# ZikangXiong/mobrob

Measured on AMD Instinct MI355X. Metric: env-steps/sec (whole node), doggo PPO, higher is better.
Workload: dtype f32

## Files before the change

mobrob_amd/csrc/engine.hip:

```cpp
#include <hip/hip_runtime.h>
#include <rccl/rccl.h>
#include <dlfcn.h>

#include <algorithm>
#include <atomic>
#include <thread>
#include <cmath>
#include <cstdarg>
#include <cstdio>
#include <climits>
#include <cstring>
#include <ctime>
#include <cstdlib>
#include <string>
#include <vector>

#ifdef MOBROB_POISON_LDS
namespace mobrob {
__global__ __launch_bounds__(1024) void k_poison_lds() {
  extern __shared__ unsigned poison_words[];
  volatile unsigned* w = poison_words;
  for (int i = threadIdx.x; i < 160 * 256; i += 1024) w[i] = 0xFFFFFFFFu;
}
inline void poison_lds(hipStream_t st) {
// ... 155 lines not shown
  ncclComm_t comm = nullptr;
  int64_t allreduce_calls = 0, allreduce_bytes = 0;
  struct OneShot {
    char* xbuf = nullptr;
    size_t payload = 0;
    char* peer[kOneShotMaxRanks] = {nullptr};
    int world = 0, rank = -1;
    bool ready = false;
    unsigned long long seq = 0;
    int* error = nullptr;
    long long timeout_ticks = 0;
  } oneshot;
  double* norm_rec_sum = nullptr; int* norm_rec_t = nullptr; int* fold_idx_dev = nullptr;
  int fold_start[kMaxTensors + 1] = {0};
  bool use_norm_records = false;
  bool epoch_kernel_on = true;
  unsigned* epoch_bar = nullptr;
  float* epoch_consts = nullptr;
  int* epoch_idx = nullptr;
  char* epoch_stage = nullptr;
  int* epoch_err_host = nullptr;
  hipEvent_t epoch_ev = nullptr;
  int last_update_mode = 0;
  float* epoch_snap = nullptr;
  int rollout64_tile_max = 256;
  int pair64_min_tiles = 65;
  int split64_max_tiles = 64;
  float *Xg = nullptr, *actg = nullptr, *lpg = nullptr, *advg = nullptr, *retg = nullptr, *oldvg = nullptr;
  float *hp[kMaxHidden] = {nullptr}, *hv[kMaxHidden] = {nullptr}, *mu = nullptr, *vout = nullptr;
  float *dmu = nullptr, *dv = nullptr, *dzp[kMaxHidden] = {nullptr}, *dzv[kMaxHidden] = {nullptr};
// ... 205 lines not shown
                       int M, int Nn, int rows, GemmQueue* q = nullptr) {
  GemmOp o;
  GemmArgs& g = o.g;
  g.A = dY; g.B = X; g.C = dW; g.M = M; g.N = Nn; g.K = rows; g.lda = ldd; g.ldb = ldx; g.ldc = ldw;
  const int wtiles = cdiv(M, M <= 32 ? 32 : 64) * cdiv(Nn, (M <= 32 || Nn <= 32) ? 32 : 64);
  int ksplit = std::max(1, std::min(cdiv(rows, 64), cdiv(2048, wtiles)));
  g.kchunk = rup(cdiv(rows, ksplit), 8);
  o.ksplit = cdiv(rows, g.kchunk);
  o.mode = MODE_TN; o.epi = EPI_ATOMIC;
  if (q) q->push_back(o); else launch_op(e, o);
}

float* Pp(mobrob_ppo_engine* e, int t) { return e->params + e->offs[t]; }
float* Gp(mobrob_ppo_engine* e, int t) { return e->grads + e->offs[t]; }

void pack_x3_all(mobrob_ppo_engine* e) {
  if (e->fused.net[0].W2x == nullptr) return;
  PackX3Args a{};
  const int w1[2] = {T_PW1, T_VW1}, w2[2] = {T_PW2, T_VW2};
  int maxthreads = 0;
  for (int n = 0; n < 2; ++n) {
    const int i1 = 3 * n, i2 = 3 * n + 1, i3 = 3 * n + 2;
    a.W[i1] = Pp(e, w1[n]); a.N[i1] = FH; a.K[i1] = e->D; a.ld[i1] = e->D; a.NB[i1] = FH / 32; a.KS[i1] = e->Dp / 16; a.scale[i1] = kTanhScale;
    a.out[i1] = reinterpret_cast<unsigned short*>(const_cast<unsigned*>(e->fused.net[n].W1x));
    a.W[i2] = Pp(e, w2[n]); a.N[i2] = FH; a.K[i2] = FH; a.ld[i2] = FH; a.NB[i2] = FH / 32; a.KS[i2] = FH / 16; a.scale[i2] = kTanhScale;
    a.out[i2] = reinterpret_cast<unsigned short*>(const_cast<unsigned*>(e->fused.net[n].W2x));
    a.W[i3] = Pp(e, w2[n]); a.N[i3] = FH; a.K[i3] = FH; a.ld[i3] = FH; a.NB[i3] = FH / 32; a.KS[i3] = FH / 16; a.scale[i3] = 1.0f; a.trans[i3] = 1;
    a.out[i3] = reinterpret_cast<unsigned short*>(const_cast<unsigned*>(e->fused.net[n].W2bx));
    maxthreads = std::max(maxthreads, std::max(a.NB[i1] * a.KS[i1], a.NB[i2] * a.KS[i2]) * 512);
  }
  hipLaunchKernelGGL(k_pack_x3_multi, dim3(cdiv(maxthreads, 256), 6), dim3(256), 0, e->stream, a);
  if (e->fused.train_chain) {
    ChainPackArgs c{};
    const int w3[2] = {T_AW, T_VW};
    for (int n = 0; n < 2; ++n) {
      c.W1[n] = Pp(e, w1[n]); c.W2[n] = Pp(e, w2[n]); c.W3[n] = Pp(e, w3[n]);
      c.w1c[n] = reinterpret_cast<unsigned short*>(const_cast<unsigned*>(e->fused.net[n].W1c));
      c.w2c[n] = reinterpret_cast<unsigned short*>(const_cast<unsigned*>(e->fused.net[n].W2c));
      c.w2bc[n] = reinterpret_cast<unsigned short*>(const_cast<unsigned*>(e->fused.net[n].W2bc));
      c.w3c[n] = const_cast<float*>(e->fused.net[n].W3c); c.w3bc[n] = const_cast<float*>(e->fused.net[n].W3bc);
      c.head[n] = n == 0 ? e->A : 1;
    }
    c.D = e->D; c.Dp = e->Dp;
    hipLaunchKernelGGL(k_pack_chain, dim3(FH * FH / 256, 2), dim3(256), 0, e->stream, c);
  }
}

void repack(mobrob_ppo_engine* e) {
  auto pad = [&](const float* src, float* dst, int r, int c, int rp, int cp) {
    hipLaunchKernelGGL(k_pad_rows, dim3(cdiv(rp * cp, 256)), dim3(256), 0, e->stream, src, dst, r, c, rp, cp);
  };
  pad(Pp(e, T_PW1), e->pW1p, e->H1, e->D, e->H1, e->Dp);
  pad(Pp(e, T_VW1), e->vW1p, e->G1, e->D, e->G1, e->Dp);
  pad(Pp(e, T_AW), e->aWp, e->A, e->HL, e->Ap, e->HL);
  pad(Pp(e, T_VW), e->vWp, 1, e->GL, 8, e->GL);
  fused_repack(e->fused, e->params, e->offs, e->stream);
  pack_x3_all(e);
}

void forward_generic(mobrob_ppo_engine* e, const float* X, int rows, bool want_pi, float* mu_out, bool want_v,
                     float* v_out, bool keep_z = false) {
  GemmQueue qp, qv;
  if (want_pi) {
    linear_fwd(e, X, e->Dp, e->pW1p, e->Dp, Pp(e, e->tPB[0]), e->hp[0], e->Hp[0], rows, e->Hp[0], e->Dp, true, keep_z ? e->dzp[0] : nullptr, &qp);
    for (int l = 1; l < e->Lp; ++l)
      linear_fwd(e, e->hp[l - 1], e->Hp[l - 1], Pp(e, e->tPW[l]), e->Hp[l - 1], Pp(e, e->tPB[l]), e->hp[l], e->Hp[l], rows, e->Hp[l], e->Hp[l - 1], true,
                 keep_z ? e->dzp[l] : nullptr, &qp);
    linear_fwd(e, e->hp[e->Lp - 1], e->HL, e->aWp, e->HL, Pp(e, T_AB), mu_out, e->Ap, rows, e->A, e->HL, false, nullptr, &qp);
  }
  if (want_v) {
    linear_fwd(e, X, e->Dp, e->vW1p, e->Dp, Pp(e, e->tVB[0]), e->hv[0], e->Hv[0], rows, e->Hv[0], e->Dp, true, keep_z ? e->dzv[0] : nullptr, &qv);
    for (int l = 1; l < e->Lv; ++l)
      linear_fwd(e, e->hv[l - 1], e->Hv[l - 1], Pp(e, e->tVW[l]), e->Hv[l - 1], Pp(e, e->tVB[l]), e->hv[l], e->Hv[l], rows, e->Hv[l], e->Hv[l - 1], true,
                 keep_z ? e->dzv[l] : nullptr, &qv);
    linear_fwd(e, e->hv[e->Lv - 1], e->GL, e->vWp, e->GL, Pp(e, T_VB), v_out, 1, rows, 1, e->GL, false, nullptr, &qv);
  }
  run_queues(e, qp, qv, 1);
}

void forward(mobrob_ppo_engine* e, const float* X, int rows, bool want_pi, float* mu_out, bool want_v, float* v_out) {
  if (e->fused.enabled && fused_forward(e->fused, X, rows, want_pi, mu_out, e->Ap, want_v, v_out, e->stream)) return;
  forward_generic(e, X, rows, want_pi, mu_out, want_v, v_out);
}

int value_net_width_sum(const mobrob_ppo_engine* e) {
  int s = 0;
  for (int l = 0; l < e->Lv; ++l) s += e->Hv[l];
  return s;
}
ValueNetArgs value_net_args(mobrob_ppo_engine* e) {
  ValueNetArgs vn{};
  for (int l = 0; l < e->Lv; ++l) { vn.W[l] = Pp(e, e->tVW[l]); vn.b[l] = Pp(e, e->tVB[l]); vn.G[l] = e->Hv[l]; }
  vn.Wv = Pp(e, T_VW); vn.bv = Pp(e, T_VB);
  vn.L = e->Lv; vn.act = e->cfg.activation; vn.width_sum = value_net_width_sum(e);
  return vn;
// ... 19 lines not shown
void sde_resample(mobrob_ppo_engine* e, int r0, int n, uint32_t draw, const uint32_t* draw_base, bool single) {
  const int HLA = e->HL * e->A, per = cdiv(HLA, 4);
  hipLaunchKernelGGL(k_sde_resample, dim3(cdiv((n + (single ? 1 : 0)) * per, 256)), dim3(256), 0, e->stream, Pp(e, T_LOGSTD), HLA, e->A, e->sde_mode, r0, n,
                     eps_seed(e) ^ 0x5DE5DE5DE5DE5DEull, draw, draw_base, e->sde_E, single ? e->sde_E1 : (float*)nullptr);
}

void sde_variance(mobrob_ppo_engine* e, int rows, bool fresh_table, float* lat2 = nullptr) {
  if (fresh_table)
    hipLaunchKernelGGL(k_sde_std2, dim3(cdiv(e->HL * e->A, 256)), dim3(256), 0, e->stream, Pp(e, T_LOGSTD), e->HL, e->A, e->sde_mode, e->sde_S2);
  hipLaunchKernelGGL(k_sde_var, dim3(cdiv(rows, 4)), dim3(256), 0, e->stream, e->hp[e->Lp - 1], e->HL, e->sde_S2, rows, e->HL, e->A, e->sde_var, e->Ap,
                     lat2);
}

void act_rows(mobrob_ppo_engine* e, int t, int r0, int n, const float* eps_dev_or_null, uint32_t draw,
              const uint32_t* draw_base, float* clip_out = nullptr) {
  ProfScope ps(e, MOBROB_K_ACT);
  if (!clip_out) clip_out = e->clip_act + (size_t)r0 * e->A;
  const size_t row = (size_t)t * e->N + r0;
  const float* X = e->obs + row * e->Dp;
  if (e->fused.enabled) {
    FusedActArgs a{};
    a.X = X; a.rows = n; a.row0 = r0; a.want_pi = 1; a.want_v = 1; a.mu = nullptr; a.ldmu = e->Ap;
    a.v = e->values + row; a.sample = 1; a.A = e->A; a.log_std = Pp(e, T_LOGSTD); a.eps = eps_dev_or_null;
    a.seed = eps_seed(e); a.draw = draw; a.draw_base = draw_base; a.lo = (float)e->cfg.action_low; a.hi = (float)e->cfg.action_high;
    a.act_raw = e->actions + row * e->A; a.act_clip = clip_out; a.logp = e->logp + row;
    fused_launch_act(e->fused, a, e->stream);
    return;
  }
  forward(e, X, n, true, e->mu, true, e->values + row);
  if (e->sde) {
// ... 45 lines not shown
  return a;
}
template <class Args>
Args reduce_args(const mobrob_ppo_engine* e) {
  Args s{};
  s.slabs = e->fused.slabs; s.grads = e->grads; s.P = e->P;
  for (int i = 0; i < 14; ++i) s.offs[i] = e->offs[i];
  s.D = e->D; s.A = e->A; s.ent_coef = (float)e->cfg.ent_coef; s.sums = e->grads + e->P;
  s.rec_sum = e->use_norm_records ? e->norm_rec_sum : nullptr; s.rec_t = e->norm_rec_t;
  return s;
}
Slab64ReduceArgs slab64_reduce_args(const mobrob_ppo_engine* e) { return reduce_args<Slab64ReduceArgs>(e); }
SlabReduceArgs slab_reduce_args(const mobrob_ppo_engine* e) {
  SlabReduceArgs s = reduce_args<SlabReduceArgs>(e);
  s.slab_floats = e->fused.slab_floats; s.Dp = e->Dp; s.h16 = e->A <= 16;
  return s;
}
StatsArgs stats_args(const mobrob_ppo_engine* e) {
  StatsArgs st{};
  st.loss_sums = e->grads + e->P; st.log_std = e->params + e->offs[T_LOGSTD]; st.n_act = e->A; st.sde = e->sde;
  st.ent_coef = (float)e->cfg.ent_coef; st.vf_coef = (float)e->cfg.vf_coef;
  return st;
}
int fused_carve_packs(mobrob_ppo_engine* e) {
  FusedState& f = e->fused;
  const int H = f.H;
  const size_t nW1 = (size_t)(H / 32) * (e->Dp / 8) * 256, nW2 = (size_t)(H / 32) * (H / 8) * 256;
  const size_t nW3f = (size_t)(H / 8) * 256, nW3b = (size_t)(H / 32) * 4 * 256;
  const size_t nW3h = (size_t)(H / 16) * 256;
  const size_t per_net = nW1 + 2 * nW2 + nW3f + nW3h + nW3b + 2 * H;
// ... 59 lines not shown
        f.lds_chain_bytes = chain_lds_bytes(e->Dp);
      }
    }
    CHK(dalloc(e, &f.train_rec, (size_t)e->N * e->T * train_rec_width(e->A)));
    f.lds_bytes = fused_lds_bytes(e->Dp);
    f.lds_act_bytes = fused_lds_act_bytes(e->Dp);
  }
  return dalloc(e, &f.stamps, 32);
}
int build_norm_record_tables(mobrob_ppo_engine* e) {
  const FusedState& f = e->fused;
  const int nb = cdiv(f.slab_floats, 256);
  CHK(dalloc(e, &e->norm_rec_sum, (size_t)2 * nb * kNormRec));
  CHK(dalloc(e, &e->norm_rec_t, (size_t)2 * nb * kNormRec));
  CHK(dalloc(e, &e->fold_idx_dev, (size_t)2 * nb * kNormRec));
  const SlabReduceArgs s256 = slab_reduce_args(e);
  const Slab64ReduceArgs s64 = slab64_reduce_args(e);
  std::vector<std::vector<int>> per_tensor(13);
  for (int net = 0; net < 2; ++net)
    for (int b = 0; b < nb; ++b) {
      std::vector<int> recs;
      for (int w = 0; w < 4; ++w) {
        std::vector<int> wave;
        for (int l = 0; l < 64; ++l) {
          const int p = b * 256 + w * 64 + l;
          const int dst = p < f.slab_floats ? (f.H == 64 ? slab64_to_canonical(s64, net, p) : slab_to_canonical(s256, net, p)) : -1;
          const int t = tensor_of_canonical(e->offs, e->P, dst);
          if (t >= 0 && std::find(wave.begin(), wave.end(), t) == wave.end()) wave.push_back(t);
        }
        for (int t : wave)
// ... 826 lines not shown
}
int rollout_side_stream_init(mobrob_ppo_engine* e) {
  if (!e->vstream) {
    HIPC(hipStreamCreateWithFlags(&e->vstream, hipStreamNonBlocking));
    HIPC(hipEventCreateWithFlags(&e->ev_vdone, hipEventDisableTiming));
  }
  while ((int)e->ev_chunks.size() < e->T / 16 + 2) {
    hipEvent_t ev;
    HIPC(hipEventCreateWithFlags(&ev, hipEventDisableTiming));
    e->ev_chunks.push_back(ev);
  }
  return MOBROB_OK;
}

RolloutArgs rollout_args(mobrob_ppo_engine* e) {
  RolloutArgs a{};
  a.pi = e->fused.net[0];
  a.log_std = Pp(e, T_LOGSTD); a.seed = eps_seed(e);
  a.lo = (float)e->cfg.action_low; a.hi = (float)e->cfg.action_high;
  a.bt = BootArgs{Pp(e, T_VW1), Pp(e, T_VB1), Pp(e, T_VW2), Pp(e, T_VB2), Pp(e, T_VW), Pp(e, T_VB), e->G1, e->G2,
                  (float)e->cfg.gamma, e->term_val};
  a.N = e->N; a.D = e->D; a.A = e->A;
  a.obs = e->obs; a.actions = e->actions; a.logp = e->logp; a.rewards = e->rewards; a.es = e->es;
  a.term_obs = e->term_obs; a.trunc = e->trunc_dev; a.clip_act = e->clip_act;
  a.ep_len = e->ep_len; a.prev_dones = e->prev_dones; a.gstate = e->gstate[0]; a.ep_stats = e->ep_stats;
  return a;
}

bool wide_nets(const mobrob_ppo_engine* e) { return e->fused.H == FH; }
bool rollout64_tile_kernel(const mobrob_ppo_engine* e) { return cdiv(e->N, 32) <= e->rollout64_tile_max; }
// ... 144 lines not shown
    if (sp.kind == 1) {
      hipLaunchKernelGGL(k_env_reset, dim3(cdiv(N * per, 256)), dim3(256), 0, e->stream, env_seed_of(e), N, e->D, Dp, last,
                         e->ep_len);
    } else {
      hipLaunchKernelGGL(k_goal_env_reset, dim3(cdiv(N * per, 256)), dim3(256), 0, e->stream, env_seed_of(e), N, e->D, Dp,
                         sp.goal, e->gstate[0], last);
      HIPC(hipMemsetAsync(e->ep_stats, 0, kEpStatsDoubles * sizeof(double), e->stream));
      e->ep_ring_read = 0;
    }
    std::vector<float> ones(N, 1.0f);
    HIPC(hipMemcpyAsync(e->prev_dones, ones.data(), (size_t)N * 4, hipMemcpyHostToDevice, e->stream));
    HIPC(hipStreamSynchronize(e->stream));
    e->env_started = sp.kind;
  }
  e->rollout_ready = false; e->train_rec_valid = false;
  if (rollout_persistent_ok(e)) CHK(rollout_side_stream_init(e));
  bool use_graph = e->cfg.rollout_graph && e->T % 2 == 0 && !rollout_persistent_ok(e);
  if (use_graph && (e->ro_exec == nullptr || memcmp(&e->ro_spec, &sp, sizeof sp) != 0)) {
    HIPC(hipStreamSynchronize(e->stream));
    if (e->ro_exec) { (void)hipGraphExecDestroy(e->ro_exec); e->ro_exec = nullptr; }
    if (e->ro_graph) { (void)hipGraphDestroy(e->ro_graph); e->ro_graph = nullptr; }
    const bool prof = e->prof_on;
    e->prof_on = false;
    hipError_t be = hipStreamBeginCapture(e->stream, hipStreamCaptureModeThreadLocal);
    if (be != hipSuccess) {
      (void)hipGetLastError();
      e->prof_on = prof;
      e->cfg.rollout_graph = 0;
      use_graph = false;
    } else {
// ... 466 lines not shown
  if (!e->fused.enabled) generic_minibatch_grad(e, mb, start, B, inv_bg);
  else if (e->fused.H == 64) fused64_minibatch_grad(e, mb, start, B, inv_bg);
  else fused_minibatch_grad(e, mb, start, B, inv_bg);
  HIPC(hipGetLastError());
  e->grad_pending = true;
  return MOBROB_OK;
}

namespace {
void fill_adam_pack_args(mobrob_ppo_engine* e, AdamPackArgs& a) {
  a.p = e->params; a.g = e->grads; a.m = e->m; a.v = e->v; a.P = e->P;
  a.chunks = e->chunks_dev; a.partial = e->chunk_partial; a.nchunks = e->nchunks;
  if (e->use_norm_records) {
    a.partial = e->norm_rec_sum; a.fold_idx = e->fold_idx_dev;
    for (int i = 0; i <= kMaxTensors; ++i) a.fold_start[i] = e->fold_start[i];
  }
  a.max_norm = (float)e->cfg.max_grad_norm; a.beta1 = (float)e->cfg.adam_beta1; a.beta2 = (float)e->cfg.adam_beta2;
  a.eps = (float)e->cfg.adam_eps;
  for (int i = 0; i <= kMaxTensors; ++i) a.offs[i] = e->offs[i];
  a.ntens = e->ntens; a.two_by_two = e->Lp == 2 && e->Lv == 2; a.id_pw1 = T_PW1; a.id_vw1 = T_VW1; a.id_aw = T_AW; a.id_vw = T_VW; a.HL = e->HL; a.GL = e->GL;
  a.D = e->D; a.Dp = e->Dp; a.A = e->A; a.Ap = e->Ap; a.H1 = e->H1; a.H2 = e->H2; a.G1 = e->G1; a.G2 = e->G2;
  a.pW1p = e->pW1p; a.vW1p = e->vW1p; a.aWp = e->aWp; a.vWp = e->vWp;
  for (int n = 0; n < 2; ++n) {
    const bool on = e->fused.enabled;
    a.fW1f[n] = on ? (float*)e->fused.net[n].W1f : nullptr;
    a.fW2f[n] = on ? (float*)e->fused.net[n].W2f : nullptr;
    a.fW3f[n] = on ? (float*)e->fused.net[n].W3f : nullptr;
    const bool ch = on && e->fused.train_chain;
    a.fW2b[n] = on && !ch ? (float*)e->fused.net[n].W2b : nullptr;
    a.fW3b[n] = on && !ch ? (float*)e->fused.net[n].W3b : nullptr;
    a.fW3h[n] = (on && (n == 1 || e->fused.A <= 16)) ? (float*)e->fused.net[n].W3h : nullptr;
    a.fb1s[n] = on ? (float*)e->fused.net[n].b1s : nullptr;
    a.fb2s[n] = on ? (float*)e->fused.net[n].b2s : nullptr;
    const bool x3 = on && e->fused.train_x3;
    a.xW1[n] = x3 ? reinterpret_cast<unsigned short*>(const_cast<unsigned*>(e->fused.net[n].W1x)) : nullptr;
    a.xW2[n] = x3 ? reinterpret_cast<unsigned short*>(const_cast<unsigned*>(e->fused.net[n].W2x)) : nullptr;
    a.xW2b[n] = x3 && !ch ? reinterpret_cast<unsigned short*>(const_cast<unsigned*>(e->fused.net[n].W2bx)) : nullptr;
    a.cW1[n] = ch ? reinterpret_cast<unsigned short*>(const_cast<unsigned*>(e->fused.net[n].W1c)) : nullptr;
    a.cW2[n] = ch ? reinterpret_cast<unsigned short*>(const_cast<unsigned*>(e->fused.net[n].W2c)) : nullptr;
    a.cW2b[n] = ch ? reinterpret_cast<unsigned short*>(const_cast<unsigned*>(e->fused.net[n].W2bc)) : nullptr;
    a.cW3[n] = ch ? const_cast<float*>(e->fused.net[n].W3c) : nullptr;
    a.cW3b[n] = ch ? const_cast<float*>(e->fused.net[n].W3bc) : nullptr;
  }
}
}

namespace {
struct AdamStep { float step_size, bc2_sqrt; };
AdamStep next_adam_step(mobrob_ppo_engine* e) {
  e->adam_step++;
  const double bc1 = 1.0 - std::pow(e->cfg.adam_beta1, (double)e->adam_step), bc2 = 1.0 - std::pow(e->cfg.adam_beta2, (double)e->adam_step);
// ... 9 lines not shown
  st.inv_bg = 1.0f / (float)((int64_t)e->cur_count * e->cfg.world_size);
  if (!e->use_norm_records)
    hipLaunchKernelGGL(k_sqnorm_chunks, dim3(e->nchunks), dim3(256), 0, e->stream, e->grads, e->chunks_dev,
                       e->chunk_partial, st);
  return st;
}
int apply_adam(mobrob_ppo_engine* e, const StatsArgs& st) {
  const AdamStep step = next_adam_step(e);
  AdamPackArgs a{};
  fill_adam_pack_args(e, a);
  a.step_size = step.step_size; a.bc2_sqrt = step.bc2_sqrt;
  if (e->use_norm_records) a.st = st;
  a.stats_row = st.stats_row;
  a.loss_sums_zero = e->fused.enabled ? e->grads + e->P : nullptr;
  hipLaunchKernelGGL(k_adam_pack, dim3(cdiv(e->P, 256)), dim3(256), 0, e->stream, a);
  HIPC(hipGetLastError());
  e->grad_pending = false;
  return MOBROB_OK;
}
}

namespace {
int apply_checked(mobrob_ppo_engine* e, int32_t* stopped) {
  *stopped = 0;
  ProfScope ps(e, MOBROB_K_APPLY);
  const StatsArgs st = apply_norms(e);
  if (e->target_kl > 0.0) {
    float approx_kl = 0.f;
    HIPC(hipMemcpyAsync(&approx_kl, st.stats_row + 4, sizeof(float), hipMemcpyDeviceToHost, e->stream));
    HIPC(hipStreamSynchronize(e->stream));
// ... 253 lines not shown
  e->last_steps_applied += nmb;
  return MOBROB_OK;
}

int train_loop(mobrob_ppo_engine* e, const int64_t* perms, bool dp, bool records, mobrob_allreduce_fn fn, void* ctx) {
  if (!dp && e->cfg.world_size != 1)
    return fail(MOBROB_ERR_STATE, "mobrob_ppo_train is the single-rank loop; data-parallel ranks call mobrob_ppo_train_dp "
                                  "(or drive epoch_begin/minibatch_grad/[all-reduce]/minibatch_apply)");
  const size_t total = (size_t)e->N * e->T;
  e->stats_n = 0;
  const bool kl = e->target_kl > 0.0;
  e->last_epochs_started = 0; e->last_stopped_early = 0; e->last_steps_applied = 0;
  struct RecordsOn {
    mobrob_ppo_engine* e;
    RecordsOn(mobrob_ppo_engine* e_, bool on) : e(e_) { e->use_norm_records = on; }
    ~RecordsOn() { e->use_norm_records = false; }
  } records_on(e, records);
  EpochLaunch epoch_launch;
  const bool epoch_kernel = epoch_kernel_eligible(e, dp, records, &epoch_launch);
  e->last_update_mode = epoch_kernel ? 1 : 0;
  for (int ep = 0; ep < e->cfg.n_epochs; ++ep) {
    CHK(mobrob_ppo_epoch_begin(e, perms ? perms + (size_t)ep * total : nullptr));
    if (dp) CHK(dp_all_reduce(e, e->advstat, (size_t)e->nmb * 4, 1, fn, ctx));
    e->last_epochs_started = ep + 1;
    if (ep == e->cfg.n_epochs - 1 || kl) e->stats_n = 0;
    if (epoch_kernel) {
      CHK(launch_epoch_kernel(e, ep, epoch_launch));
      continue;
    }
    for (int mb = 0; mb < e->nmb && !e->last_stopped_early; ++mb) {
      CHK(mobrob_ppo_minibatch_grad(e, mb));
// ... 768 lines not shown
```

mobrob_amd/csrc/kernels_fused.h:

```cpp
#pragma once
#include "device_utils.h"

namespace mobrob {

constexpr int FH = 256;
constexpr int FR = 64;
constexpr int FLDH = FH + 4;
constexpr int FLDO = 36;
constexpr int FTHREADS = 256;

struct FusedNet {
  const f32x4* W1f;
  const f32x4* W2f;
  const f32x4* W3f;
  const f32x4* W3h;
  const f32x4* W2b;
  const f32x4* W3b;
  const float* b1s; const float* b2s;
  const float* b3;
  int head;
  const unsigned* W1x;
  const unsigned* W2x;
  const unsigned* W2bx;
  const unsigned* W1c;
// ... 1415 lines not shown
    __syncthreads();
    if (tid < 4)
      slab[slab_off_st(DP) + tid] = (lds[L::STAT + tid] + lds[L::STAT + 4 + tid]) + (lds[L::STAT + 8 + tid] + lds[L::STAT + 12 + tid]);
  }
}

struct SlabReduceArgs {
  const float* slabs; int slab_floats; int nslabs;
  float* grads; int P;
  int offs[14];
  int D, Dp, A;
  int h16;
  float ent_coef, b_local, inv_bg;
  float* sums;
  double* rec_sum; int* rec_t;
};

constexpr int kNormRec = 4;
template <class PI>
__host__ __device__ inline int tensor_of_canonical(PI offs, int P, int dst) {
  if (dst < 0 || dst >= P) return -1;
  int t = 0;
  for (int k = 1; k < 13; ++k) t += (dst >= offs[k]) ? 1 : 0;
  return t;
}
template <bool COH = false>
__device__ __forceinline__ void block_norm_records(int t, float val, double* rec_sum, int* rec_t) {
  __shared__ double sc[4 * kNormRec];
  __shared__ int sct[4 * kNormRec];
  const int lane = threadIdx.x & 63, wave = threadIdx.x >> 6;
// ... 16 lines not shown
    int n = 0, cur = -1;
    double acc = 0.0;
    for (int k = 0; k < 4 * kNormRec; ++k) {
      const int tt = sct[k];
      if (tt < 0) continue;
      if (tt == cur) { acc += sc[k]; continue; }
      if (cur >= 0 && n < kNormRec) { stc<COH>(rec_sum + n, acc); stc<COH>(rec_t + n, cur); ++n; }
      cur = tt;
      acc = sc[k];
    }
    if (cur >= 0 && n < kNormRec) { stc<COH>(rec_sum + n, acc); stc<COH>(rec_t + n, cur); ++n; }
    for (; n < kNormRec; ++n) stc<COH>(rec_t + n, -1);
  }
}

__host__ __device__ __forceinline__ int slab_to_canonical(const SlabReduceArgs& s, int net, int p) {
  const int T_W1 = net == 0 ? 1 : 5, T_B1 = net == 0 ? 2 : 6, T_W2 = net == 0 ? 3 : 7, T_B2 = net == 0 ? 4 : 8;
  const int T_W3 = net == 0 ? 9 : 11, T_B3 = net == 0 ? 10 : 12;
  const int head = net == 0 ? s.A : 1;
  auto frag = [](int q, int nt, int* w, int* t, int* i, int* lane) {
    *lane = (q >> 2) & 63;
    *i = (q & 3) + 4 * ((q >> 8) & 3);
    const int wt = q >> 10;
    *t = wt % nt;
    *w = wt / nt;
  };
  int w, t, i, lane;
  if (p < slab_off_w1()) {
    frag(p, 16, &w, &t, &i, &lane);
    const int n = 64 * w + 32 * (t >> 3) + crc(i) + 4 * (lane >> 5), j = 32 * (t & 7) + (lane & 31);
// ... 59 lines not shown
    }
#pragma unroll
    for (int k = 0; k < U; ++k)
      if (w + k < n) ac[k] += src[(size_t)(w + k) * stride];
#pragma unroll
    for (int d = U / 2; d >= 1; d >>= 1)
#pragma unroll
      for (int k = 0; k < d; ++k) ac[k] += ac[k + d];
    acc = ac[0];
    if (dst < s.offs[1]) acc = __fadd_rn(acc, __fmul_rn(__fmul_rn(s.ent_coef, -s.b_local), s.inv_bg));
    s.grads[dst] = acc;
  }
  if (s.rec_sum != nullptr) {
    const size_t b = ((size_t)net * gridDim.x + blockIdx.x) * kNormRec;
    block_norm_records(tensor_of_canonical(s.offs, s.P, dst), acc, s.rec_sum + b, s.rec_t + b);
  }
}

__global__ void k_pack_fwd(const float* __restrict__ W, int N, int K, int ld, float* __restrict__ out, int NB,
                           int KG, float scale) {
  const int i = blockIdx.x * blockDim.x + threadIdx.x;
  if (i >= NB * KG * 256) return;
  const int s = i & 3, lane = (i >> 2) & 63, kg = (i >> 8) % KG, nb = (i >> 8) / KG;
  const int n = nb * 32 + (lane & 31), k = kg * 8 + 4 * (lane >> 5) + s;
  out[i] = (n < N && k < K) ? scale * W[(size_t)n * ld + k] : 0.f;
}
__host__ __device__ inline int pack_h16_idx(int n, int k) { return (((k >> 4) * 64) + 16 * ((k >> 2) & 3) + n) * 4 + (k & 3); }
__global__ void k_pack_h16(const float* __restrict__ W, int N, int K, float* __restrict__ out) {
  const int i = blockIdx.x * blockDim.x + threadIdx.x;
  if (i >= (K / 16) * 256) return;
// ... 263 lines not shown
__global__ __launch_bounds__(256) void k_sqnorm_chunks(const float* __restrict__ g, const NormChunk* __restrict__ chunks,
                                                       double* __restrict__ partial, StatsArgs st) {
  __shared__ double sc[16];
  if (blockIdx.x == 0 && threadIdx.x == 0 && st.stats_row != nullptr) stats_row_from_sums(st, entropy_of_log_std(st.log_std, st.n_act));
  const double tot = block_sum_d(chunk_sumsq_thread(g, chunks[blockIdx.x], threadIdx.x), sc);
  if (threadIdx.x == 0) partial[blockIdx.x] = tot;
}

constexpr int kMaxTensors = 1 + 4 * kMaxHidden + 4;
constexpr int kFusedTensors = 17;
struct AdamPackArgs {
  float* p; const float* g; float* m; float* v; int P;
  float* g_out;
  const NormChunk* chunks; const double* partial; int nchunks;
  const int* fold_idx; int fold_start[kMaxTensors + 1];
  float max_norm, step_size, bc2_sqrt, beta1, beta2, eps;
  int offs[kMaxTensors + 1];
  int ntens;
  int two_by_two;
  int id_pw1, id_vw1, id_aw, id_vw;
  int HL, GL;
  int D, Dp, A, Ap, H1, H2, G1, G2;
  float* pW1p; float* vW1p; float* aWp; float* vWp;
  float* fW1f[2]; float* fW2f[2]; float* fW3f[2]; float* fW3h[2]; float* fW2b[2]; float* fW3b[2]; float* fb1s[2]; float* fb2s[2];
  unsigned short* xW1[2]; unsigned short* xW2[2]; unsigned short* xW2b[2];
  unsigned short* cW1[2]; unsigned short* cW2[2]; unsigned short* cW2b[2]; float* cW3[2]; float* cW3b[2];
  float* stats_row;
  float* loss_sums_zero;
  StatsArgs st;
};
// ... 35 lines not shown
  out[base + 1024] = (unsigned short)(p3 & 0xffffu);
}
__device__ __forceinline__ void chain_store_w1(unsigned short* w1c, int n, int k, int K1, float scaled) {
  chain_pack_store(w1c, chain_pack_idx(chain_unit_w1(n >> 4, k >> 5, K1), n, (k >> 3) & 3, k & 7), scaled);
}
__device__ __forceinline__ void chain_store_w2(unsigned short* w2c, unsigned short* w2bc, int n, int k, float scaled, float raw) {
  int s, g, j;
  chain_kslot_of_neuron(k, &s, &g, &j);
  chain_pack_store(w2c, chain_pack_idx(chain_unit_w2(n >> 4, s), n, g, j), scaled);
  chain_kslot_of_neuron(n, &s, &g, &j);
  chain_pack_store(w2bc, chain_pack_idx(chain_unit_w2b(k >> 4, s), k, g, j), raw);
}
__host__ __device__ __forceinline__ int chain_head_fwd_idx(int a_, int k) { return ((k >> 4) * 64 + a_ + 16 * ((k >> 2) & 3)) * 4 + (k & 3); }
__host__ __device__ __forceinline__ int chain_head_bwd_idx(int a_, int k) { return ((k >> 4) * 64 + (k & 15) + 16 * (a_ >> 2)) * 4 + (a_ & 3); }

template <bool COH = false, class TA = AdamPackArgs>
__device__ __forceinline__ void adam_pack_apply(const TA& a, int i, float graw, float m0, float v0, float p0, float coef, float step_size, float bc2_sqrt) {
  const float g = __fmul_rn(graw, coef);
  const float m = __fmaf_rn(g, 1.0f - a.beta1, __fmul_rn(m0, a.beta1));
  const float v = __fmaf_rn(__fmul_rn(g, g), 1.0f - a.beta2, __fmul_rn(v0, a.beta2));
  const float denom = __fadd_rn(__fdiv_rn(__fsqrt_rn(v), bc2_sqrt), a.eps);
  const float pn = __fmaf_rn(-step_size, __fdiv_rn(m, denom), p0);
  int t = 0;
#pragma unroll
  for (int k = 1; k < kFusedTensors; ++k) t += (i >= a.offs[k]) ? 1 : 0;
  if (a.ntens > kFusedTensors)
    for (int k = kFusedTensors; k < a.ntens; ++k) t += (i >= a.offs[k]) ? 1 : 0;
  const int e = i - a.offs[t];
  a.m[i] = m;
  a.v[i] = v;
// ... 3 lines not shown
  return;
#endif
  if (!a.two_by_two) {
    if (t == a.id_pw1 || t == a.id_vw1) {
      const int n = e / a.D, k = e - n * a.D;
      (t == a.id_vw1 ? a.vW1p : a.pW1p)[n * a.Dp + k] = pn;
    } else if (t == a.id_aw || t == a.id_vw) {
      (t == a.id_vw ? a.vWp : a.aWp)[e] = pn;
    }
    return;
  }
  switch (t) {
    case 1: case 5: {
      const int net = t == 5, n = e / a.D, k = e - n * a.D;
      (net ? a.vW1p : a.pW1p)[n * a.Dp + k] = pn;
      if (a.fW1f[net]) stc<COH>(a.fW1f[net] + pack_fwd_idx(n, k, a.Dp / 8), kTanhScale * pn);
      if (a.xW1[net]) x3_pack_store(a.xW1[net], n, k, a.Dp / 16, kTanhScale * pn);
      if (a.cW1[net]) chain_store_w1(a.cW1[net], n, k, (a.Dp + 31) / 32, kTanhScale * pn);
    } break;
    case 3: case 7: {
      const int net = t == 7;
      if (a.fW2f[net]) {
        const int K = net ? a.G1 : a.H1, n = e / K, k = e - n * K;
        stc<COH>(a.fW2f[net] + pack_fwd_idx(n, k, K / 8), kTanhScale * pn);
        if (a.fW2b[net]) stc<COH>(a.fW2b[net] + pack_bwd_idx(n, k, (net ? a.G2 : a.H2) / 8), pn);
        if (a.xW2[net]) x3_pack_store(a.xW2[net], n, k, K / 16, kTanhScale * pn);
        if (a.xW2b[net]) x3_pack_store(a.xW2b[net], k, n, (net ? a.G2 : a.H2) / 16, pn);
        if (a.cW2[net]) chain_store_w2(a.cW2[net], a.cW2b[net], n, k, kTanhScale * pn, pn);
      }
    } break;
    case 9: case 11: {
      const int net = t == 11, K = net ? a.G2 : a.H2, n = e / K, k = e - n * K;
      (net ? a.vWp : a.aWp)[e] = pn;
      if (a.fW3f[net]) {
        stc<COH>(a.fW3f[net] + pack_fwd_idx(n, k, K / 8), pn);
        if (a.fW3b[net]) stc<COH>(a.fW3b[net] + pack_bwd_idx(n, k, 4), pn);
        if (a.fW3h[net] && n < 16) stc<COH>(a.fW3h[net] + pack_h16_idx(n, k), pn);
        if (a.cW3[net] && n < 16) { a.cW3[net][chain_head_fwd_idx(n, k)] = pn; a.cW3b[net][chain_head_bwd_idx(n, k)] = pn; }
      }
    } break;
    case 2: case 6: if (a.fb1s[t == 6]) stc<COH>(a.fb1s[t == 6] + e, kTanhScale * pn); break;
    case 4: case 8: if (a.fb2s[t == 8]) stc<COH>(a.fb2s[t == 8] + e, kTanhScale * pn); break;
    default: break;
  }
}

template <bool COH, class TA>
__device__ __forceinline__ void adam_pack_block_at(const TA& a, int lin, int i, float g_in, float m_in, float v_in, float p_in, float step_size,
                                                   float bc2_sqrt, float* stats_row, float inv_bg, float ent_pre, int fidx_pre = -1) {
  __shared__ double part[1024];
  __shared__ int tens[256];
  __shared__ float nts[kMaxTensors + 3];
  __shared__ float coef_s, total_s;
  if (lin == 0 && a.st.loss_sums != nullptr) {
    StatsArgs st;
    st.stats_row = stats_row; st.loss_sums = a.st.loss_sums; st.log_std = a.st.log_std;
    st.ent_coef = a.st.ent_coef; st.vf_coef = a.st.vf_coef; st.inv_bg = inv_bg; st.n_act = a.st.n_act; st.sde = a.st.sde;
    stats_row_from_sums<COH>(st, ent_pre);
  }
  if (a.fold_idx != nullptr) {
    const int nrec = a.fold_start[13];
    if (nrec <= 128) {
      if ((int)threadIdx.x < nrec) part[threadIdx.x] = ldc<COH>(a.partial + (fidx_pre >= 0 ? fidx_pre : a.fold_idx[threadIdx.x]));
      __syncthreads();
      if (threadIdx.x < 13) {
        double ts = 0.0;
        for (int c = a.fold_start[threadIdx.x]; c < a.fold_start[threadIdx.x + 1]; ++c) ts += part[c];
        nts[threadIdx.x] = (float)sqrt(ts);
      }
    } else {
      const int lane = threadIdx.x & 63, wv = threadIdx.x >> 6;
      const bool staged = nrec <= 1024;
      if (staged) {
        for (int c = threadIdx.x; c < nrec; c += blockDim.x) part[c] = ldc<COH>(a.partial + a.fold_idx[c]);
        __syncthreads();
      }
      for (int t = wv; t < 13; t += 4) {
        double ts = 0.0;
        if (staged)
          for (int c = a.fold_start[t] + lane; c < a.fold_start[t + 1]; c += 64) ts += part[c];
        else
          for (int c = a.fold_start[t] + lane; c < a.fold_start[t + 1]; c += 64) ts += ldc<COH>(a.partial + a.fold_idx[c]);
        ts = wave_sum_d(ts);
        if (lane == 0) nts[t] = (float)sqrt(ts);
      }
    }
  } else {
    for (int c = threadIdx.x; c < a.nchunks; c += blockDim.x) {
      part[c] = ldc<COH>(a.partial + c);
      tens[c] = a.chunks[c].tensor;
    }
    __syncthreads();
    if ((int)threadIdx.x < a.ntens) {
      double ts = 0.0;
      for (int c = 0; c < a.nchunks; ++c)
        if (tens[c] == (int)threadIdx.x) ts += part[c];
      nts[threadIdx.x] = (float)sqrt(ts);
    }
  }
  __syncthreads();
  if (threadIdx.x == 0) {
    float tot_sq = 0.f;
    for (int t = 0; t < a.ntens; ++t) tot_sq = __fmaf_rn(nts[t], nts[t], tot_sq);
    const float total = sqrtf(tot_sq);
    total_s = total;
    coef_s = fminf(a.max_norm / (total + 1e-6f), 1.0f);
  }
  __syncthreads();
  const float coef = coef_s;
  if (lin == 0 && stats_row != nullptr) stats_row[6] = total_s;
  if (lin < 8 && a.loss_sums_zero != nullptr) stc<COH>(a.loss_sums_zero + lin, 0.f);
  if (i < 0 || i >= a.P) return;
  adam_pack_apply<COH>(a, i, g_in, m_in, v_in, p_in, coef, step_size, bc2_sqrt);
}
template <bool COH, class TA>
__device__ __forceinline__ void adam_pack_block(const TA& a, int bx, float step_size, float bc2_sqrt, float* stats_row, float inv_bg) {
  const int i = bx * 256 + (int)threadIdx.x;
  float g_in = 0.f, m_in = 0.f, v_in = 0.f, p_in = 0.f;
  if (i < a.P) { g_in = ldc<COH>(a.g + i); m_in = ldc<COH>(a.m + i); v_in = ldc<COH>(a.v + i); p_in = ldc<COH>(a.p + i); }
  const float ent = (i == 0 && a.st.loss_sums != nullptr) ? entropy_of_log_std<COH>(a.st.log_std, a.st.n_act) : 0.f;
  adam_pack_block_at<COH>(a, i, i, g_in, m_in, v_in, p_in, step_size, bc2_sqrt, stats_row, inv_bg, ent);
}
__global__ __launch_bounds__(256) void k_adam_pack(AdamPackArgs a) {
  adam_pack_block<false>(a, blockIdx.x, a.step_size, a.bc2_sqrt, a.stats_row, a.st.inv_bg);
}
// ... 69 lines not shown
```

Measured before the change: 31.89 million.

## Compute grad-clip coefficient once via last-block ticket and defer rollout weight packs

The slab reduce kernel now uses an atomic ticket so the last block folds the per-tensor norm records and publishes the global norm and clip coefficient. Every Adam block then reads that value instead of each recomputing the fold. Separately, when the train chain is active, Adam steps skip writing the rollout-only packed weight layouts on every minibatch. Those packs are marked dirty and rebuilt once before the next forward or rollout. This cuts redundant per-block reductions and scattered stores during training, at the cost of an extra repack pass and new cross-block atomic ordering that must be correct.

```diff
diff --git a/mobrob_amd/csrc/engine.hip b/mobrob_amd/csrc/engine.hip
--- a/mobrob_amd/csrc/engine.hip
+++ b/mobrob_amd/csrc/engine.hip
@@ -193,6 +193,10 @@
   double* norm_rec_sum = nullptr; int* norm_rec_t = nullptr; int* fold_idx_dev = nullptr;
   int fold_start[kMaxTensors + 1] = {0};
   bool use_norm_records = false;
+  float* clip_pub = nullptr;
+  bool clip_ticket_on = true;
+  bool defer_packs_on = true;
+  bool rollout_packs_dirty = false;
   bool epoch_kernel_on = true;
   unsigned* epoch_bar = nullptr;
   float* epoch_consts = nullptr;
@@ -428,7 +432,7 @@
 float* Pp(mobrob_ppo_engine* e, int t) { return e->params + e->offs[t]; }
 float* Gp(mobrob_ppo_engine* e, int t) { return e->grads + e->offs[t]; }
 
-void pack_x3_all(mobrob_ppo_engine* e) {
+void pack_x3_all(mobrob_ppo_engine* e, bool chain_too = true) {
   if (e->fused.net[0].W2x == nullptr) return;
   PackX3Args a{};
   const int w1[2] = {T_PW1, T_VW1}, w2[2] = {T_PW2, T_VW2};
@@ -444,7 +448,7 @@
     maxthreads = std::max(maxthreads, std::max(a.NB[i1] * a.KS[i1], a.NB[i2] * a.KS[i2]) * 512);
   }
   hipLaunchKernelGGL(k_pack_x3_multi, dim3(cdiv(maxthreads, 256), 6), dim3(256), 0, e->stream, a);
-  if (e->fused.train_chain) {
+  if (chain_too && e->fused.train_chain) {
     ChainPackArgs c{};
     const int w3[2] = {T_AW, T_VW};
     for (int n = 0; n < 2; ++n) {
@@ -470,6 +474,13 @@
   pad(Pp(e, T_VW), e->vWp, 1, e->GL, 8, e->GL);
   fused_repack(e->fused, e->params, e->offs, e->stream);
   pack_x3_all(e);
+  e->rollout_packs_dirty = false;
+}
+void flush_rollout_packs(mobrob_ppo_engine* e) {
+  if (!e->rollout_packs_dirty) return;
+  fused_repack(e->fused, e->params, e->offs, e->stream);
+  pack_x3_all(e, false);
+  e->rollout_packs_dirty = false;
 }
 
 void forward_generic(mobrob_ppo_engine* e, const float* X, int rows, bool want_pi, float* mu_out, bool want_v,
@@ -493,6 +504,7 @@
 }
 
 void forward(mobrob_ppo_engine* e, const float* X, int rows, bool want_pi, float* mu_out, bool want_v, float* v_out) {
+  flush_rollout_packs(e);
   if (e->fused.enabled && fused_forward(e->fused, X, rows, want_pi, mu_out, e->Ap, want_v, v_out, e->stream)) return;
   forward_generic(e, X, rows, want_pi, mu_out, want_v, v_out);
 }
@@ -542,6 +554,7 @@
 
 void act_rows(mobrob_ppo_engine* e, int t, int r0, int n, const float* eps_dev_or_null, uint32_t draw,
               const uint32_t* draw_base, float* clip_out = nullptr) {
+  flush_rollout_packs(e);
   ProfScope ps(e, MOBROB_K_ACT);
   if (!clip_out) clip_out = e->clip_act + (size_t)r0 * e->A;
   const size_t row = (size_t)t * e->N + r0;
@@ -617,6 +630,11 @@
 SlabReduceArgs slab_reduce_args(const mobrob_ppo_engine* e) {
   SlabReduceArgs s = reduce_args<SlabReduceArgs>(e);
   s.slab_floats = e->fused.slab_floats; s.Dp = e->Dp; s.h16 = e->A <= 16;
+  if (s.rec_sum != nullptr && e->clip_ticket_on) {
+    s.clip = e->clip_pub; s.ticket = reinterpret_cast<unsigned*>(e->clip_pub + 2);
+    s.fold_idx = e->fold_idx_dev; s.max_norm = (float)e->cfg.max_grad_norm;
+    for (int i = 0; i < 14; ++i) s.fold_start[i] = e->fold_start[i];
+  }
   return s;
 }
 StatsArgs stats_args(const mobrob_ppo_engine* e) {
@@ -706,6 +724,9 @@
   CHK(dalloc(e, &e->norm_rec_sum, (size_t)2 * nb * kNormRec));
   CHK(dalloc(e, &e->norm_rec_t, (size_t)2 * nb * kNormRec));
   CHK(dalloc(e, &e->fold_idx_dev, (size_t)2 * nb * kNormRec));
+  CHK(dalloc(e, &e->clip_pub, 4));
+  e->clip_ticket_on = !env_switched_off("MOBROB_NO_CLIP_TICKET");
+  e->defer_packs_on = !env_switched_off("MOBROB_NO_DEFER_PACKS");
   const SlabReduceArgs s256 = slab_reduce_args(e);
   const Slab64ReduceArgs s64 = slab64_reduce_args(e);
   std::vector<std::vector<int>> per_tensor(13);
@@ -1562,6 +1583,7 @@
 }
 
 RolloutArgs rollout_args(mobrob_ppo_engine* e) {
+  flush_rollout_packs(e);
   RolloutArgs a{};
   a.pi = e->fused.net[0];
   a.log_std = Pp(e, T_LOGSTD); a.seed = eps_seed(e);
@@ -1736,6 +1758,7 @@
     e->env_started = sp.kind;
   }
   e->rollout_ready = false; e->train_rec_valid = false;
+  flush_rollout_packs(e);
   if (rollout_persistent_ok(e)) CHK(rollout_side_stream_init(e));
   bool use_graph = e->cfg.rollout_graph && e->T % 2 == 0 && !rollout_persistent_ok(e);
   if (use_graph && (e->ro_exec == nullptr || memcmp(&e->ro_spec, &sp, sizeof sp) != 0)) {
@@ -2232,6 +2255,7 @@
   if (e->use_norm_records) {
     a.partial = e->norm_rec_sum; a.fold_idx = e->fold_idx_dev;
     for (int i = 0; i <= kMaxTensors; ++i) a.fold_start[i] = e->fold_start[i];
+    if (e->fused.H == FH && e->clip_ticket_on) a.clip_in = e->clip_pub;
   }
   a.max_norm = (float)e->cfg.max_grad_norm; a.beta1 = (float)e->cfg.adam_beta1; a.beta2 = (float)e->cfg.adam_beta2;
   a.eps = (float)e->cfg.adam_eps;
@@ -2241,18 +2265,19 @@
   a.pW1p = e->pW1p; a.vW1p = e->vW1p; a.aWp = e->aWp; a.vWp = e->vWp;
   for (int n = 0; n < 2; ++n) {
     const bool on = e->fused.enabled;
-    a.fW1f[n] = on ? (float*)e->fused.net[n].W1f : nullptr;
-    a.fW2f[n] = on ? (float*)e->fused.net[n].W2f : nullptr;
-    a.fW3f[n] = on ? (float*)e->fused.net[n].W3f : nullptr;
     const bool ch = on && e->fused.train_chain;
+    const bool defer = ch && e->defer_packs_on;
     a.fW2b[n] = on && !ch ? (float*)e->fused.net[n].W2b : nullptr;
     a.fW3b[n] = on && !ch ? (float*)e->fused.net[n].W3b : nullptr;
-    a.fW3h[n] = (on && (n == 1 || e->fused.A <= 16)) ? (float*)e->fused.net[n].W3h : nullptr;
+    a.fW1f[n] = on && !defer ? (float*)e->fused.net[n].W1f : nullptr;
+    a.fW2f[n] = on && !defer ? (float*)e->fused.net[n].W2f : nullptr;
+    a.fW3f[n] = on && !defer ? (float*)e->fused.net[n].W3f : nullptr;
+    a.fW3h[n] = (on && !defer && (n == 1 || e->fused.A <= 16)) ? (float*)e->fused.net[n].W3h : nullptr;
     a.fb1s[n] = on ? (float*)e->fused.net[n].b1s : nullptr;
     a.fb2s[n] = on ? (float*)e->fused.net[n].b2s : nullptr;
     const bool x3 = on && e->fused.train_x3;
-    a.xW1[n] = x3 ? reinterpret_cast<unsigned short*>(const_cast<unsigned*>(e->fused.net[n].W1x)) : nullptr;
-    a.xW2[n] = x3 ? reinterpret_cast<unsigned short*>(const_cast<unsigned*>(e->fused.net[n].W2x)) : nullptr;
+    a.xW1[n] = x3 && !defer ? reinterpret_cast<unsigned short*>(const_cast<unsigned*>(e->fused.net[n].W1x)) : nullptr;
+    a.xW2[n] = x3 && !defer ? reinterpret_cast<unsigned short*>(const_cast<unsigned*>(e->fused.net[n].W2x)) : nullptr;
     a.xW2b[n] = x3 && !ch ? reinterpret_cast<unsigned short*>(const_cast<unsigned*>(e->fused.net[n].W2bx)) : nullptr;
     a.cW1[n] = ch ? reinterpret_cast<unsigned short*>(const_cast<unsigned*>(e->fused.net[n].W1c)) : nullptr;
     a.cW2[n] = ch ? reinterpret_cast<unsigned short*>(const_cast<unsigned*>(e->fused.net[n].W2c)) : nullptr;
@@ -2292,6 +2317,7 @@
   a.stats_row = st.stats_row;
   a.loss_sums_zero = e->fused.enabled ? e->grads + e->P : nullptr;
   hipLaunchKernelGGL(k_adam_pack, dim3(cdiv(e->P, 256)), dim3(256), 0, e->stream, a);
+  if (e->fused.enabled && e->fused.train_chain && e->defer_packs_on) e->rollout_packs_dirty = true;
   HIPC(hipGetLastError());
   e->grad_pending = false;
   return MOBROB_OK;
@@ -2575,7 +2601,7 @@
   struct RecordsOn {
     mobrob_ppo_engine* e;
     RecordsOn(mobrob_ppo_engine* e_, bool on) : e(e_) { e->use_norm_records = on; }
-    ~RecordsOn() { e->use_norm_records = false; }
+    ~RecordsOn() { e->use_norm_records = false; flush_rollout_packs(e); }
   } records_on(e, records);
   EpochLaunch epoch_launch;
   const bool epoch_kernel = epoch_kernel_eligible(e, dp, records, &epoch_launch);
diff --git a/mobrob_amd/csrc/kernels_fused.h b/mobrob_amd/csrc/kernels_fused.h
--- a/mobrob_amd/csrc/kernels_fused.h
+++ b/mobrob_amd/csrc/kernels_fused.h
@@ -1453,6 +1453,7 @@
   float ent_coef, b_local, inv_bg;
   float* sums;
   double* rec_sum; int* rec_t;
+  unsigned* ticket; float* clip; const int* fold_idx; int fold_start[14]; float max_norm;
 };
 
 constexpr int kNormRec = 4;
@@ -1499,6 +1500,43 @@
   }
 }
 
+template <bool COH, class FS>
+__device__ __forceinline__ void fold_norm_records(const double* partial, const int* fold_idx, const FS& fold_start, int fidx_pre, double* part, float* nts) {
+  const int nrec = fold_start[13];
+  if (nrec <= 128) {
+    if ((int)threadIdx.x < nrec) part[threadIdx.x] = ldc<COH>(partial + (fidx_pre >= 0 ? fidx_pre : fold_idx[threadIdx.x]));
+    __syncthreads();
+    if (threadIdx.x < 13) {
+      double ts = 0.0;
+      for (int c = fold_start[threadIdx.x]; c < fold_start[threadIdx.x + 1]; ++c) ts += part[c];
+      nts[threadIdx.x] = (float)sqrt(ts);
+    }
+  } else {
+    const int lane = threadIdx.x & 63, wv = threadIdx.x >> 6;
+    const bool staged = nrec <= 1024;
+    if (staged) {
+      for (int c = threadIdx.x; c < nrec; c += blockDim.x) part[c] = ldc<COH>(partial + fold_idx[c]);
+      __syncthreads();
+    }
+    for (int t = wv; t < 13; t += 4) {
+      double ts = 0.0;
+      if (staged)
+        for (int c = fold_start[t] + lane; c < fold_start[t + 1]; c += 64) ts += part[c];
+      else
+        for (int c = fold_start[t] + lane; c < fold_start[t + 1]; c += 64) ts += ldc<COH>(partial + fold_idx[c]);
+      ts = wave_sum_d(ts);
+      if (lane == 0) nts[t] = (float)sqrt(ts);
+    }
+  }
+}
+__device__ __forceinline__ void clip_from_norms(const float* nts, int ntens, float max_norm, float* total_out, float* coef_out) {
+  float tot_sq = 0.f;
+  for (int t = 0; t < ntens; ++t) tot_sq = __fmaf_rn(nts[t], nts[t], tot_sq);
+  const float total = sqrtf(tot_sq);
+  *total_out = total;
+  *coef_out = fminf(max_norm / (total + 1e-6f), 1.0f);
+}
+
 __host__ __device__ __forceinline__ int slab_to_canonical(const SlabReduceArgs& s, int net, int p) {
   const int T_W1 = net == 0 ? 1 : 5, T_B1 = net == 0 ? 2 : 6, T_W2 = net == 0 ? 3 : 7, T_B2 = net == 0 ? 4 : 8;
   const int T_W3 = net == 0 ? 9 : 11, T_B3 = net == 0 ? 10 : 12;
@@ -1588,6 +1626,26 @@
   if (s.rec_sum != nullptr) {
     const size_t b = ((size_t)net * gridDim.x + blockIdx.x) * kNormRec;
     block_norm_records(tensor_of_canonical(s.offs, s.P, dst), acc, s.rec_sum + b, s.rec_t + b);
+    if (s.ticket != nullptr) {
+      __shared__ double part[1024];
+      __shared__ float nts[16];
+      __shared__ int last_s;
+      if (threadIdx.x == 0) {
+        const unsigned nblk = gridDim.x * gridDim.y;
+        last_s = __hip_atomic_fetch_add(s.ticket, 1u, __ATOMIC_ACQ_REL, __HIP_MEMORY_SCOPE_AGENT) == nblk - 1u;
+      }
+      __syncthreads();
+      if (last_s) {
+        fold_norm_records<true>(s.rec_sum, s.fold_idx, s.fold_start, -1, part, nts);
+        __syncthreads();
+        if (threadIdx.x == 0) {
+          float total, coef;
+          clip_from_norms(nts, 13, s.max_norm, &total, &coef);
+          s.clip[0] = total; s.clip[1] = coef;
+          __hip_atomic_store(s.ticket, 0u, __ATOMIC_RELAXED, __HIP_MEMORY_SCOPE_AGENT);
+        }
+      }
+    }
   }
 }
 
@@ -1881,6 +1939,7 @@
   float* g_out;
   const NormChunk* chunks; const double* partial; int nchunks;
   const int* fold_idx; int fold_start[kMaxTensors + 1];
+  const float* clip_in;
   float max_norm, step_size, bc2_sqrt, beta1, beta2, eps;
   int offs[kMaxTensors + 1];
   int ntens;
@@ -1946,6 +2005,10 @@
 __host__ __device__ __forceinline__ int chain_head_fwd_idx(int a_, int k) { return ((k >> 4) * 64 + a_ + 16 * ((k >> 2) & 3)) * 4 + (k & 3); }
 __host__ __device__ __forceinline__ int chain_head_bwd_idx(int a_, int k) { return ((k >> 4) * 64 + (k & 15) + 16 * (a_ >> 2)) * 4 + (a_ & 3); }
 
+#ifndef MOBROB_TAIL_ABLATE
+#define MOBROB_TAIL_ABLATE 0
+#endif
+constexpr bool kAblateRolloutPacks = (MOBROB_TAIL_ABLATE & 2) != 0;
 template <bool COH = false, class TA = AdamPackArgs>
 __device__ __forceinline__ void adam_pack_apply(const TA& a, int i, float graw, float m0, float v0, float p0, float coef, float step_size, float bc2_sqrt) {
   const float g = __fmul_rn(graw, coef);
@@ -1979,30 +2042,26 @@
     case 1: case 5: {
       const int net = t == 5, n = e / a.D, k = e - n * a.D;
       (net ? a.vW1p : a.pW1p)[n * a.Dp + k] = pn;
-      if (a.fW1f[net]) stc<COH>(a.fW1f[net] + pack_fwd_idx(n, k, a.Dp / 8), kTanhScale * pn);
-      if (a.xW1[net]) x3_pack_store(a.xW1[net], n, k, a.Dp / 16, kTanhScale * pn);
+      if (!kAblateRolloutPacks && a.fW1f[net]) stc<COH>(a.fW1f[net] + pack_fwd_idx(n, k, a.Dp / 8), kTanhScale * pn);
+      if (!kAblateRolloutPacks && a.xW1[net]) x3_pack_store(a.xW1[net], n, k, a.Dp / 16, kTanhScale * pn);
       if (a.cW1[net]) chain_store_w1(a.cW1[net], n, k, (a.Dp + 31) / 32, kTanhScale * pn);
     } break;
     case 3: case 7: {
       const int net = t == 7;
-      if (a.fW2f[net]) {
-        const int K = net ? a.G1 : a.H1, n = e / K, k = e - n * K;
-        stc<COH>(a.fW2f[net] + pack_fwd_idx(n, k, K / 8), kTanhScale * pn);
-        if (a.fW2b[net]) stc<COH>(a.fW2b[net] + pack_bwd_idx(n, k, (net ? a.G2 : a.H2) / 8), pn);
-        if (a.xW2[net]) x3_pack_store(a.xW2[net], n, k, K / 16, kTanhScale * pn);
-        if (a.xW2b[net]) x3_pack_store(a.xW2b[net], k, n, (net ? a.G2 : a.H2) / 16, pn);
-        if (a.cW2[net]) chain_store_w2(a.cW2[net], a.cW2b[net], n, k, kTanhScale * pn, pn);
-      }
+      const int K = net ? a.G1 : a.H1, n = e / K, k = e - n * K;
+      if (!kAblateRolloutPacks && a.fW2f[net]) stc<COH>(a.fW2f[net] + pack_fwd_idx(n, k, K / 8), kTanhScale * pn);
+      if (a.fW2b[net]) stc<COH>(a.fW2b[net] + pack_bwd_idx(n, k, (net ? a.G2 : a.H2) / 8), pn);
+      if (!kAblateRolloutPacks && a.xW2[net]) x3_pack_store(a.xW2[net], n, k, K / 16, kTanhScale * pn);
+      if (a.xW2b[net]) x3_pack_store(a.xW2b[net], k, n, (net ? a.G2 : a.H2) / 16, pn);
+      if (a.cW2[net]) chain_store_w2(a.cW2[net], a.cW2b[net], n, k, kTanhScale * pn, pn);
     } break;
     case 9: case 11: {
       const int net = t == 11, K = net ? a.G2 : a.H2, n = e / K, k = e - n * K;
       (net ? a.vWp : a.aWp)[e] = pn;
-      if (a.fW3f[net]) {
-        stc<COH>(a.fW3f[net] + pack_fwd_idx(n, k, K / 8), pn);
-        if (a.fW3b[net]) stc<COH>(a.fW3b[net] + pack_bwd_idx(n, k, 4), pn);
-        if (a.fW3h[net] && n < 16) stc<COH>(a.fW3h[net] + pack_h16_idx(n, k), pn);
-        if (a.cW3[net] && n < 16) { a.cW3[net][chain_head_fwd_idx(n, k)] = pn; a.cW3b[net][chain_head_bwd_idx(n, k)] = pn; }
-      }
+      if (!kAblateRolloutPacks && a.fW3f[net]) stc<COH>(a.fW3f[net] + pack_fwd_idx(n, k, K / 8), pn);
+      if (a.fW3b[net]) stc<COH>(a.fW3b[net] + pack_bwd_idx(n, k, 4), pn);
+      if (!kAblateRolloutPacks && a.fW3h[net] && n < 16) stc<COH>(a.fW3h[net] + pack_h16_idx(n, k), pn);
+      if (a.cW3[net] && n < 16) { a.cW3[net][chain_head_fwd_idx(n, k)] = pn; a.cW3b[net][chain_head_bwd_idx(n, k)] = pn; }
     } break;
     case 2: case 6: if (a.fb1s[t == 6]) stc<COH>(a.fb1s[t == 6] + e, kTanhScale * pn); break;
     case 4: case 8: if (a.fb2s[t == 8]) stc<COH>(a.fb2s[t == 8] + e, kTanhScale * pn); break;
@@ -2023,57 +2082,37 @@
     st.ent_coef = a.st.ent_coef; st.vf_coef = a.st.vf_coef; st.inv_bg = inv_bg; st.n_act = a.st.n_act; st.sde = a.st.sde;
     stats_row_from_sums<COH>(st, ent_pre);
   }
-  if (a.fold_idx != nullptr) {
-    const int nrec = a.fold_start[13];
-    if (nrec <= 128) {
-      if ((int)threadIdx.x < nrec) part[threadIdx.x] = ldc<COH>(a.partial + (fidx_pre >= 0 ? fidx_pre : a.fold_idx[threadIdx.x]));
+  float coef, total;
+#if MOBROB_TAIL_ABLATE & 1
+  coef = 1.0f; total = 0.f;
+  __syncthreads();
+#else
+  if (a.clip_in != nullptr) {
+    total = a.clip_in[0]; coef = a.clip_in[1];
+    __syncthreads();
+  } else {
+    if (a.fold_idx != nullptr) {
+      fold_norm_records<COH>(a.partial, a.fold_idx, a.fold_start, fidx_pre, part, nts);
+    } else {
+      for (int c = threadIdx.x; c < a.nchunks; c += blockDim.x) {
+        part[c] = ldc<COH>(a.partial + c);
+        tens[c] = a.chunks[c].tensor;
+      }
       __syncthreads();
-      if (threadIdx.x < 13) {
+      if ((int)threadIdx.x < a.ntens) {
         double ts = 0.0;
-        for (int c = a.fold_start[threadIdx.x]; c < a.fold_start[threadIdx.x + 1]; ++c) ts += part[c];
+        for (int c = 0; c < a.nchunks; ++c)
+          if (tens[c] == (int)threadIdx.x) ts += part[c];
         nts[threadIdx.x] = (float)sqrt(ts);
       }
-    } else {
-      const int lane = threadIdx.x & 63, wv = threadIdx.x >> 6;
-      const bool staged = nrec <= 1024;
-      if (staged) {
-        for (int c = threadIdx.x; c < nrec; c += blockDim.x) part[c] = ldc<COH>(a.partial + a.fold_idx[c]);
-        __syncthreads();
-      }
-      for (int t = wv; t < 13; t += 4) {
-        double ts = 0.0;
-        if (staged)
-          for (int c = a.fold_start[t] + lane; c < a.fold_start[t + 1]; c += 64) ts += part[c];
-        else
-          for (int c = a.fold_start[t] + lane; c < a.fold_start[t + 1]; c += 64) ts += ldc<COH>(a.partial + a.fold_idx[c]);
-        ts = wave_sum_d(ts);
-        if (lane == 0) nts[t] = (float)sqrt(ts);
-      }
-    }
-  } else {
-    for (int c = threadIdx.x; c < a.nchunks; c += blockDim.x) {
-      part[c] = ldc<COH>(a.partial + c);
-      tens[c] = a.chunks[c].tensor;
     }
     __syncthreads();
-    if ((int)threadIdx.x < a.ntens) {
-      double ts = 0.0;
-      for (int c = 0; c < a.nchunks; ++c)
-        if (tens[c] == (int)threadIdx.x) ts += part[c];
-      nts[threadIdx.x] = (float)sqrt(ts);
-    }
-  }
-  __syncthreads();
-  if (threadIdx.x == 0) {
-    float tot_sq = 0.f;
-    for (int t = 0; t < a.ntens; ++t) tot_sq = __fmaf_rn(nts[t], nts[t], tot_sq);
-    const float total = sqrtf(tot_sq);
-    total_s = total;
-    coef_s = fminf(a.max_norm / (total + 1e-6f), 1.0f);
-  }
-  __syncthreads();
-  const float coef = coef_s;
-  if (lin == 0 && stats_row != nullptr) stats_row[6] = total_s;
+    if (threadIdx.x == 0) clip_from_norms(nts, a.ntens, a.max_norm, &total_s, &coef_s);
+    __syncthreads();
+    coef = coef_s; total = total_s;
+  }
+#endif
+  if (lin == 0 && stats_row != nullptr) stats_row[6] = total;
   if (lin < 8 && a.loss_sums_zero != nullptr) stc<COH>(a.loss_sums_zero + lin, 0.f);
   if (i < 0 || i >= a.P) return;
   adam_pack_apply<COH>(a, i, g_in, m_in, v_in, p_in, coef, step_size, bc2_sqrt);
```

Result: slower. 30.75 million (-3.6%).
